# samyak0210/ViNet

Measured on AMD Instinct MI355X. Metric: clips/sec training (32x224x384 bf16), higher is better.
Workload: dtype bf16; 1 GPU; ViNet DHF1K training, 32x224x384 bf16, 192 clip(s)/GPU/step, kldiv + fused Adam, 1xMI355X; global_batch=192, local_batch=192, parallelism=dp1

## Files before the change

include/vinet_hip.h:

```cpp
#ifndef VINET_HIP_H
#define VINET_HIP_H

#include <stddef.h>
#include <stdint.h>

#ifdef __cplusplus
extern "C" {
#endif

#define VINET_ABI_VERSION 16

enum { VINET_F32 = 0, VINET_BF16 = 1,
       VINET_F32S = 2 };
enum { VINET_ACT_NONE = 0, VINET_ACT_RELU = 1, VINET_ACT_SIGMOID = 2 };
enum { VINET_CONV_GENERIC = 0, VINET_CONV_STEM = 1 };

typedef struct VinetTensor {
  void* ptr;
  int32_t B, T, H, W, C;
  int32_t ld;
  int64_t sB;
} VinetTensor;

typedef struct VinetAffine {
// ... 50 lines not shown
  VinetTensor x;
  VinetTensor dy;
  int32_t sT, sH, sW;
  int32_t ntaps;
  const int32_t* taps;
  float* dw;
  int32_t Kp;
  VinetAffine pre;
  int32_t tline;
  int32_t tpad;
  const void* bnb_z;
  int32_t bnb_ld;
  int64_t bnb_sB;
  VinetAffine bnb_fwd;
  const float* bnb_mean;
  const float* bnb_invstd;
  const float* bnb_c1;
  const float* bnb_c2;
  int32_t max_cus;
} VinetWgradDesc;

int vinet_conv3d_wgrad(const VinetWgradDesc* desc, void* stream);
int vinet_conv3d_wgrad_fuses_bn_bwd(const VinetWgradDesc* desc);
int vinet_conv3d_wgrad_kernel_name(const VinetWgradDesc* desc, char* buf, int32_t n);

int vinet_pack_weights(const float* w, int32_t N, int32_t Cin, int32_t ntaps, int32_t transpose, int32_t stem,
                       int32_t dtype, void* out, void* stream);

int vinet_pack_weights_multi(const int64_t* table, int32_t njobs, int64_t total, int32_t dtype, void* stream);
int vinet_unpack_wgrad(float* dw, int32_t N, int32_t Cin, int32_t ntaps, int32_t stem, int32_t flags,
                       float* grad, void* stream);
int vinet_unpack_wgrad_multi(const int64_t* table, int32_t njobs, int64_t total, int32_t flags, void* stream);

int vinet_import_ncdhw(const float* src, int64_t sb, int64_t sc, int64_t st, int64_t sh, int64_t sw, int32_t C,
                       const VinetTensor* dst, int32_t dst_dtype, void* stream);
int vinet_import_ncdhw_pad(const float* src, int64_t sb, int64_t sc, int64_t st, int64_t sh, int64_t sw, int32_t C,
                           int32_t Hs, int32_t Ws, int32_t pad_top, int32_t pad_left, const VinetTensor* dst,
                           int32_t dst_dtype, void* stream);
int vinet_export_ncdhw(const VinetTensor* src, int32_t src_dtype, VinetAffine pre, float* dst, int64_t sb, int64_t sc,
                       int64_t st, int64_t sh, int64_t sw, int32_t accumulate, void* stream);
int vinet_copy_affine(const VinetTensor* src, int32_t src_dtype, VinetAffine pre, const VinetTensor* dst,
                      int32_t dst_dtype, int32_t accumulate, void* stream);

int vinet_bn_finalize(const float* partials, int32_t rows, int32_t C, int32_t ld, double count, const float* gamma,
                      const float* beta, float eps, float momentum, float* running_mean, float* running_var,
                      float* mean, float* invstd, float* scale, float* shift, void* stream);
// ... 170 lines not shown
```

vinet_amd/_lib.py:

```python
import ctypes as C
import os

HERE = os.path.dirname(os.path.abspath(__file__))
LIB_PATH = os.environ.get("VINET_LIB") or os.path.join(HERE, "libvinet_hip.so")

F32, BF16 = 0, 1
F32S = 2
ACT_NONE, ACT_RELU, ACT_SIGMOID = 0, 1, 2
CONV_GENERIC, CONV_STEM = 0, 1
TK_MMA_F32, TK_MMA_BF16X3, TK_MMA_BF16 = 0, 1, 2
ABI_VERSION = 16


class CTensor(C.Structure):
    _fields_ = [("ptr", C.c_void_p), ("B", C.c_int32), ("T", C.c_int32), ("H", C.c_int32), ("W", C.c_int32),
                ("C", C.c_int32), ("ld", C.c_int32), ("sB", C.c_int64)]


class CAffine(C.Structure):
    _fields_ = [("scale", C.c_void_p), ("shift", C.c_void_p), ("relu", C.c_int32)]


class CConvDesc(C.Structure):
    _fields_ = [("dtype", C.c_int32), ("out_dtype", C.c_int32), ("mode", C.c_int32), ("x", CTensor), ("y", CTensor),
# ... 28 lines not shown
                ("L", C.c_int32), ("train", C.c_int32), ("p", C.c_float), ("eps", C.c_float), ("seed", C.c_uint64),
                ("step", C.c_void_p), ("pe", C.c_void_p), ("params", C.POINTER(C.c_void_p)), ("grads", C.POINTER(C.c_void_p)),
                ("ws", C.c_void_p), ("ws_bytes", C.c_int64), ("masks", C.c_void_p)]


class CTokenEncoderDesc(C.Structure):
    _fields_ = list(CTransformerDesc._fields_)


_vp, _i32, _i64, _f32, _f64 = C.c_void_p, C.c_int32, C.c_int64, C.c_float, C.c_double
_PT, _PC, _PW, _PP = C.POINTER(CTensor), C.POINTER(CConvDesc), C.POINTER(CWgradDesc), C.POINTER(CPoolDesc)
_PX = C.POINTER(CTransformerDesc)
_PK = C.POINTER(CTokenEncoderDesc)

SIGNATURES = {
    "vinet_conv3d": [_PC, _vp],
    "vinet_conv3d_tile_m": [_PC],
    "vinet_conv3d_stats_rows": [_PC],
    "vinet_conv3d_applies_pre_once": [_PC],
    "vinet_conv3d_splitk_bytes": [_PC],
    "vinet_conv3d_kernel_name": [_PC, C.c_char_p, _i32],
    "vinet_conv3d_wgrad": [_PW, _vp],
    "vinet_conv3d_wgrad_kernel_name": [_PW, C.c_char_p, _i32],
    "vinet_pack_weights": [_vp, _i32, _i32, _i32, _i32, _i32, _i32, _vp, _vp],
    "vinet_unpack_wgrad": [_vp, _i32, _i32, _i32, _i32, _i32, _vp, _vp],
    "vinet_import_ncdhw": [_vp, _i64, _i64, _i64, _i64, _i64, _i32, _PT, _i32, _vp],
    "vinet_import_ncdhw_pad": [_vp, _i64, _i64, _i64, _i64, _i64, _i32, _i32, _i32, _i32, _i32, _PT, _i32, _vp],
    "vinet_export_ncdhw": [_PT, _i32, CAffine, _vp, _i64, _i64, _i64, _i64, _i64, _i32, _vp],
    "vinet_copy_affine": [_PT, _i32, CAffine, _PT, _i32, _i32, _vp],
    "vinet_bn_finalize": [_vp, _i32, _i32, _i32, _f64, _vp, _vp, _f32, _f32, _vp, _vp, _vp, _vp, _vp, _vp, _vp],
    "vinet_bn_fold": [_vp, _vp, _vp, _vp, _vp, _f32, _i32, _vp, _vp, _vp, _vp],
    "vinet_channel_stats": [_PT, _i32, _vp, _vp],
    "vinet_stats_rows": [_PT],
    "vinet_bn_bwd_reduce": [_PT, _PT, _i32, CAffine, _vp, _vp, _vp, _vp],
    "vinet_conv3d_wgrad_fuses_bn_bwd": [_PW],
    "vinet_conv3d_fuses_dgrad_phases": [_PC],
    "vinet_conv3d_bn_bwd_stats_rows": [_PC],
    "vinet_bn_partials_fold": [_vp, _i32, _i32, _vp, _i32, _vp],
    "vinet_bn_bwd_finalize": [_vp, _i32, _i32, _i32, _f64, _vp, _i32, _vp, _vp, _vp, _vp, _vp, _vp],
    "vinet_bn_bwd_apply": [_PT, _PT, _i32, CAffine, _vp, _vp, _vp, _vp, _PT, _vp],
    "vinet_bn_bwd_apply_split": [_PT, _PT, CAffine, _vp, _vp, _vp, _vp, _PT, _PT, _PT, _vp],
    "vinet_bn_bwd_pool_ok": [_PP, _PT, _PT, _PT, _i32],
    "vinet_bn_bwd_reduce_pool": [_PP, _PT, _vp, _PT, _i32, _PT, _i32, CAffine, _vp, _vp, _vp, _vp],
    "vinet_bn_bwd_apply_pool": [_PP, _PT, _vp, _PT, _i32, _PT, _i32, CAffine, _vp, _vp, _vp, _vp, _PT, _vp],
    "vinet_act_bwd": [_PT, _i32, _PT, _i32, _i32, _PT, _i32, _vp],
    "vinet_channel_sum": [_PT, _i32, _vp, _i32, _vp, _i32, _vp],
# ... 133 lines not shown
```

vinet_amd/csrc/conv_wgrad.hip:

```cpp
#include "conv_host.h"

struct WgradArgs {
  const char* x;
  const char* dy;
  float* dw;
  const int4* taps;
  const float* in_scale;
  const float* in_shift;
  int in_relu;
  int Ti, Hi, Wi, Cin, ldx;
  long sBx;
  int To, Ho, Wo, N, ldy;
  long sBy;
  int sT, sH, sW;
  int ntaps, Kp, M;
  int tilesN, tilesC, splitK, chunks_per_split, nchunks;
  int use_tr;
  FastDiv dW, dH, dT;
};

VN_DEV void wg_split_pair(float x0, float x1, uint32_t& hi, uint32_t& lo) {
  hi = cvt_pk_bf16_f32(x0, x1);
  lo = cvt_pk_bf16_f32(x0 - __uint_as_float(hi << 16), x1 - __uint_as_float(hi & 0xffff0000u));
}
// ... 225 lines not shown
}

static bool wgrad_use_dma(const VinetWgradDesc* d) {
  const bool pre_ok = !d->pre.scale || (d->pre.relu && d->pre.shift);
  return g_vinet_opt_wgrad_dma && d->dtype == VINET_BF16 && d->mode == VINET_CONV_GENERIC && pre_ok &&
         !(d->pre.relu && !d->pre.scale);
}

WgradRoute vinet_wgrad_route(const VinetWgradDesc* d) {
  if (vinet_wgrad_use_skinny(d)) return {WGRAD_SKINNY};
  if (vinet_wgrad_use_rs(d)) return {WGRAD_RS};
  if (vinet_wgrad_use_hs(d)) return {WGRAD_HS};
  if (vinet_wgrad_use_ts(d)) return {WGRAD_TS};
  if (vinet_wgrad_use_tf(d)) return {WGRAD_TF};
  if (!wgrad_use_dma(d)) return {WGRAD_GENERIC};
  return {vinet_wgrad_use_pp(d) ? WGRAD_PP : WGRAD_DMA};
}

extern "C" int vinet_conv3d_wgrad_kernel_name(const VinetWgradDesc* d, char* buf, int32_t n) {
  if (!d || !buf || n <= 0) return -1;
  const char* pre = d->pre.scale ? "pre" : "plain";
  switch (vinet_wgrad_route(d).kind) {
    case WGRAD_SKINNY: snprintf(buf, n, "wgrad_skinny_kernel"); break;
    case WGRAD_RS: snprintf(buf, n, "conv_wgrad_rs_kernel<W%d,%s>", d->dy.W, vinet_wgrad_rs_four_wave(d) ? "4w" : "8w"); break;
    case WGRAD_HS: snprintf(buf, n, d->bnb_z ? "conv_wgrad_hs_kernel<bn_bwd>" : "conv_wgrad_hs_kernel"); break;
    case WGRAD_TS: snprintf(buf, n, "conv_wgrad_ts_kernel<%s>", pre); break;
    case WGRAD_TF: snprintf(buf, n, "conv_wgrad_tf_kernel<%s>", pre); break;
    case WGRAD_PP: snprintf(buf, n, "conv_wgrad_pp_kernel<%s,%d>", pre, vinet_wgrad_pp_rows(d->dy.C)); break;
    case WGRAD_DMA: return vinet_wgrad_dma_name(d, buf, n);
    case WGRAD_GENERIC: snprintf(buf, n, "conv_wgrad_kernel<%s,%d>", d->dtype == VINET_BF16 ? "bf16" : (d->dtype == VINET_F32S ? "float/split" : "float"), d->mode); break;
  }
  return 0;
}

extern "C" int vinet_conv3d_wgrad_fuses_bn_bwd(const VinetWgradDesc* d) {
  return d && d->bnb_z && vinet_wgrad_route(d).kind == WGRAD_HS ? 1 : 0;
}

static int vinet_launch_wgrad_generic(const VinetWgradDesc* d, hipStream_t s) {
  WgradArgs a;
  a.x = (const char*)d->x.ptr; a.dy = (const char*)d->dy.ptr; a.dw = d->dw; a.taps = (const int4*)d->taps;
  a.in_scale = d->pre.scale; a.in_shift = d->pre.shift; a.in_relu = d->pre.relu;
  a.Ti = d->x.T; a.Hi = d->x.H; a.Wi = d->x.W; a.Cin = d->x.C; a.ldx = d->x.ld; a.sBx = d->x.sB;
  a.To = d->dy.T; a.Ho = d->dy.H; a.Wo = d->dy.W; a.N = d->dy.C; a.ldy = d->dy.ld; a.sBy = d->dy.sB;
  a.sT = d->sT; a.sH = d->sH; a.sW = d->sW;
  a.ntaps = d->ntaps; a.Kp = d->Kp;
  const long M = (long)d->dy.B * d->dy.T * d->dy.H * d->dy.W;
  VN_CHECK_ARG(M < (1L << 31), "wgrad: M too large");
  a.M = (int)M;
  a.tilesN = vn_div_up(a.N, 64);
  a.tilesC = vn_div_up(d->mode == VINET_CONV_STEM ? 32 : a.Cin, 64);
  a.nchunks = vn_div_up(M, 32);
  const long base_blocks = (long)a.tilesN * a.tilesC * a.ntaps;
  long sk = (2048 + base_blocks - 1) / base_blocks;
  if (sk > a.nchunks / 4) sk = a.nchunks / 4;
  if (sk < 1) sk = 1;
  if (sk > 4096) sk = 4096;
  a.chunks_per_split = vn_div_up(a.nchunks, sk);
  a.splitK = vn_div_up(a.nchunks, a.chunks_per_split);
// ... 44 lines not shown
```

vinet_amd/csrc/options.h:

```cpp
#pragma once
#define VN_OPTIONS(VN_OPT) \
  VN_OPT(dma,          1, "LDS-DMA conv kernel (conv_dma) where legal; 0 = the register-staged kernel") \
  VN_OPT(dma3,         1, "LDS-DMA kernel for the split-bf16 form (conv_dma3); 0 = the register-staged kernel") \
  VN_OPT(pp,           1, "256x256x64 ping-pong conv kernel: 0 off, 1 heuristic, 2 force, 3 / 4 force the 256- / 192-wide shape") \
  VN_OPT(pp_pw_kt,     8, "ping-pong kernel on pointwise layers from this many K tiles of 64 (16 = as for every other layer)") \
  VN_OPT(pw,           1, "pointwise streaming kernel (conv_pw) for 1x1x1 convs and their data gradients: 0 off, 1 heuristic, 2 also on small grids (tests)") \
  VN_OPT(pw_maxtn,     4, "pointwise kernel: at most this many column tiles (each re-reads x)") \
  VN_OPT(ht,           1, "halo-tile conv kernels (conv_ht): 0 off, 1 heuristic, 2 every eligible conv (tests)") \
  VN_OPT(ht3,          1, "halo-tile kernels for the split-bf16 form; 0 = conv_dma3 everywhere") \
  VN_OPT(ht_minhw,     28 * 48, "halo tiles, spatial mode: smallest H x W the heuristic takes") \
  VN_OPT(ht_t,         1, "temporal mode of the halo-tile kernel for (3,1,1) / stride-1 convs; 0 off") \
  VN_OPT(ht_t_minhw,   14 * 24, "halo tiles, temporal mode: smallest H x W the heuristic takes") \
  VN_OPT(ht_pre,       0, "halo tiles, spatial mode, on inputs with a pending BatchNorm + ReLU: 1 on") \
  VN_OPT(conv_hs,      1, "strip-streaming kernel of the folded stem (conv_hs): 0 off, 1 heuristic, 2 every eligible shape (tests)") \
  VN_OPT(conv_hs_segs, 1, "conv_hs: row segments for launches on small grids; 0 = whole strips only") \
  VN_OPT(conv_ts,      1, "frame-streaming temporal 64 -> 64 kernels (conv_ts, conv_tsd): 0 off, 1 heuristic, 2 every eligible shape (tests)") \
  VN_OPT(conv_ts_segs, 1, "conv_ts: frame segments for launches on small grids; 0 = whole patches only") \
  VN_OPT(splitk,       1, "split-K on grids that cannot fill the chip: 0 off, 1 on, n >= 2 = minimum K chunks (of 32) per split") \
  VN_OPT(sk_tile,      7, "tiles of long-K small-grid convs whose caller lends split-K scratch: bit 0 128x192, bit 1 128x128, bit 2 / 3 128x64 / 256x64") \
  VN_OPT(n64_tile,     0, "tuning: 64-wide layers on 128x64 (1) or 64x64 (2) tiles instead of 256x64") \
  VN_OPT(n64_kmax,     64, "64-wide outputs: 128-row tiles up to this many K steps of 32 (0 = never)") \
  VN_OPT(n128_tile,    0, "tuning: 128-wide layers on 128x128 (1) or 64x128 (2) tiles instead of 256x128") \
  VN_OPT(n128_kmax,    64, "128-wide outputs: 128-row tiles up to this many K steps of 32 (0 = never)") \
  VN_OPT(n192_tile,    1, "128x192 tiles for N % 192 == 0 instead of 256x96: 0 off, 1 heuristic, 2 also on small grids (tests)") \
  VN_OPT(tperm,        0, "t-fastest M-tile order (L2 reuse across temporal taps): 1 on") \
  VN_OPT(bnb_epi,      1, "BatchNorm-backward partial sums out of the shared conv epilogue; 0 = only the fused temporal data gradient") \
  VN_OPT(wgrad_dma,    1, "LDS-DMA multi-tap weight-gradient kernel where legal; 0 = the register-staged kernel") \
  VN_OPT(wgrad_tg,     0, "tuning: taps per group in the LDS-DMA weight gradient (0 = heuristic)") \
  VN_OPT(wgrad_tr,     1, "hardware transpose reads in the register-staged weight gradient; 0 = scalar LDS reads") \
  VN_OPT(wgrad_pp,     1, "256x256x64 ping-pong weight gradient: 0 off, 1 heuristic, 2 force, 3 / 4 force the 256- / 192-row tile") \
  VN_OPT(wgrad_pp_cap, 1, "the ping-pong weight gradient honours VinetWgradDesc::max_cus; 0 = always the whole chip") \
  VN_OPT(wgrad_ts,     1, "frame-streaming weight gradient of temporal 64 -> 64 convs: 0 off, 1 heuristic, 2 every eligible shape (tests)") \
  VN_OPT(wgrad_ts_cap, 0, "the frame-streaming weight gradient honours VinetWgradDesc::max_cus: 1 on") \
  VN_OPT(wgrad_hs,     1, "strip-streaming weight gradient of the folded stem: 0 off, 1 heuristic, 2 every eligible shape (tests)") \
  VN_OPT(wgrad_rs,     1, "row-streaming weight gradient of 1x3x3 convs: 0 off, 1 heuristic, 2 every eligible shape (tests)") \
  VN_OPT(wgrad_rs4,    1, "row-streaming weight gradient: the four-wave form for W = 24, 48, 32, 64, 96; 0 = the eight-wave kernels") \
  VN_OPT(wgrad_tf,     1, "temporal-tap weight gradient (wgrad_tf): 0 off, 1 heuristic, 2 every eligible shape (tests)") \
  VN_OPT(wgrad_skinny, 1, "weight gradient of pointwise convs with 8 output channels: 0 off, 1 heuristic, 2 every eligible shape (tests)") \
  VN_OPT(bn_lean,      1, "register-lean bf16 BatchNorm-backward kernels: 0 = the generic 8-channel forms, 1 = register-lean") \
  VN_OPT(bn_rows,      1024, "cap on the workgroups (= partial rows) of a channel reduction (clamped to >= 1)") \
  VN_OPT(reduce_il,    1, "channel reductions: blocks interleave rounds over one window; 0 = one contiguous range per block") \
  VN_OPT(reduce_small, 1, "tensors of <= 64 voxels take channel_reduce_small_kernel; 0 off") \
  VN_OPT(pack_tiled,   1, "LDS-tiled multi-tensor pack / unpack; 0 = the element-wise kernels") \
  VN_OPT(pool_lds,     1, "LDS halo-tile 3x3x3/s1 max-pool forward (C % 64 == 0): 0 off, 1 large tensors, 2 always") \
  VN_OPT(pool_pk,      1, "bf16: packed 32-bit-key form of the LDS halo-tile pool; 0 = the fp32-compare kernel") \
  VN_OPT(pool_twalk,   1, "T-walking 3x3x3/s1 max-pool backward: 0 off, 1 large tensors, 2 always (any value above 3 too), 3 conditional-load form.  The forward's 8-channel T-walking kernel (kT 3, sT 1) reads it too: >= 2 forces it on small tensors, 0 does NOT switch it off") \
  VN_OPT(pool_blk,     1, "strided max-pool backward per 2x2 input block; 0 off") \
  VN_OPT(up_blk,       1, "8-channel upsample kernels (forward per 2x2 output block); 0 off") \
  VN_OPT(auc_ws,       0, "AUC-Judd sorts and counts in the caller's workspace whatever the number of fixations: 1 on (tests); 0 = in LDS up to 4096 fixations") \
  VN_OPT(sauc_ws,      0, "shuffled AUC reads the other-fixation list from the caller's workspace whatever its length: 1 on (tests); 0 = staged in LDS up to 8192 locations")

#define VN_OPT_DECLARE(name, dflt, text) extern int g_vinet_opt_##name;
VN_OPTIONS(VN_OPT_DECLARE)
```

vinet_amd/csrc/wgrad_rs.hip:

```cpp
#include "conv_host.h"

__device__ __attribute__((aligned(64))) uint4 g_vinet_zero_page_rs[4];

struct WgradRsArgs {
  const char* x;
  const char* dy;
  float* dw;
  long sBx, sBy;
  int Ti, To, H, W, ldx, ldy;
  int kT, cchunks, nchunks, Kp, N, Cin;
  int items, workers;
  FastDiv dTo;
  float* dbg;
};

#ifdef VINET_CONV_TIMING
static float* g_wrs_dbg = nullptr;
extern "C" void vinet_debug_wrs_ptr(float* p) { g_wrs_dbg = p; }
#endif
VN_DEV int wrs_swz(int r) { return (((r >> 1) & 1) | (((r >> 3) & 1) << 1)) << 1; }

template <int KS>
__global__ __launch_bounds__(512, 1) void conv_wgrad_rs_kernel(const WgradRsArgs a) {
  constexpr int W = KS * 32, RP = W + 2;
  constexpr int XROW = RP * 128, DROW = W * 128;
  constexpr int NPC = W * 8;
  constexpr int PPT = (NPC + 511) / 512;
  extern __shared__ __attribute__((aligned(16))) char smem[];
  char* ring = smem;
  char* dyb = smem + 3 * XROW;
  const int tid = threadIdx.x, lane = tid & 63, wave = __builtin_amdgcn_readfirstlane(tid >> 6);
  const int groups = a.kT * a.cchunks * a.nchunks;
  const int lid = xcd_remap((int)blockIdx.x, (int)gridDim.x);
  const int grp = lid % groups, worker = lid / groups;
  const int n0 = (grp % a.nchunks) * 64;
  const int gc = grp / a.nchunks;
// ... 344 lines not shown
    }
  }
#ifdef VINET_CONV_TIMING
  if (a.dbg && (tid & 63) == 0) {
    float* o = a.dbg + ((long)blockIdx.x * 8 + wave) * 8;
    o[0] = (float)(__builtin_amdgcn_s_memtime() - tm_start); o[1] = (float)tm_pro; o[2] = (float)tm_mma; o[3] = (float)tm_b1;
    o[4] = (float)tm_wr; o[5] = (float)tm_b2; o[6] = (float)tm_steps; o[7] = (float)tm_items;
  }
#endif
  mfma_drain();
#pragma unroll
  for (int t = 0; t < 9; ++t)
#pragma unroll
    for (int i = 0; i < 2; ++i)
#pragma unroll
      for (int r = 0; r < 4; ++r) {
        const int n = (nh * 2 + i) * 16 + (lane >> 4) * 4 + r, c = c0 + ct * 16 + (lane & 15);
        if (n0 + n < a.N && c < a.Cin) atomicAdd(a.dw + ((long)(kt * 9 + t) * a.N + n0 + n) * (long)a.Kp + c, acc[t][i][r]);
      }
}

constexpr int wrs_gcd(int a, int b) { return b == 0 ? a : wrs_gcd(b, a % b); }
template <int V> struct WrsIC { static constexpr int value = V; };

template <int KS, int WW>
__global__ __launch_bounds__(256, 1) void conv_wgrad_rs4_kernel(const WgradRsArgs a) {
  constexpr int P = KS * 32, R = P / WW, RING = 2 * R + 2, U = RING / wrs_gcd(R, RING);
  static_assert(R * WW == P && R >= 1 && WW % 8 == 0, "whole rows per step, 8-position DMA pieces inside one row");
  constexpr int XROW = (WW + 2) * 128, DROW = P * 128;
  constexpr int PPT = KS;
  extern __shared__ __attribute__((aligned(16))) char smem[];
  char* ring = smem;
  char* dyb = smem + RING * XROW;
  const int tid = threadIdx.x, lane = tid & 63, ct = __builtin_amdgcn_readfirstlane(tid >> 6);
  const int groups = a.kT * a.cchunks * a.nchunks;
  const int lid = xcd_remap((int)blockIdx.x, (int)gridDim.x);
  const int grp = lid % groups, worker = lid / groups;
  const int n0 = (grp % a.nchunks) * 64;
  const int gc = grp / a.nchunks;
  const int kt = gc / a.cchunks, c0 = (gc - kt * a.cchunks) * 64;
  const int l_chunk = tid & 7;
  const int H = a.H;
  const char* zero = (const char*)g_vinet_zero_page_rs;

  int xo[PPT], yo[PPT];
  int pr_[PPT], pw0_[PPT];
#pragma unroll
  for (int j = 0; j < PPT; ++j) {
    const int pos0 = j * 32 + ct * 8, pos = pos0 + (lane >> 3);
    const int pr = pos0 / WW, pw = pos - pr * WW;
    pr_[j] = pr; pw0_[j] = pos0 - pr * WW;
    const int xc = l_chunk ^ wrs_swz(pw + 1), dc = l_chunk ^ wrs_swz(pos);
    xo[j] = (pw * a.ldx + c0 + (c0 + xc * 8 < a.Cin ? xc * 8 : 0)) * 2;
    yo[j] = (pos * a.ldy + n0 + (n0 + dc * 8 < a.N ? dc * 8 : 0)) * 2;
  }
  auto dma = [&](const char* base, int off, char* dst) {
    __builtin_amdgcn_global_load_lds((const __attribute__((address_space(1))) void*)(base + (unsigned)off),
                                     (__attribute__((address_space(3))) void*)dst, 16, 0, 0);
  };
  for (int i = tid; i < RING * 2 * 8; i += 256) {
    const int row = i / 16, side = (i >> 3) & 1, ch = i & 7;
    *(uint4*)(ring + row * XROW + (side ? (WW + 1) * 128 : 0) + ch * 16) = make_uint4(0, 0, 0, 0);
  }
  const int p = lane & 15, q = lane >> 4;
  int xs[KS][2][3], xwrap[KS][2], da[KS][2], ds[KS][2];
  const int db = (p & 3) >> 1;
#pragma unroll
  for (int ks = 0; ks < KS; ++ks)
#pragma unroll
    for (int h = 0; h < 2; ++h) {
      const int pos = ks * 32 + q * 8 + h * 4 + (p >> 2);
      const int fr = pos / WW, fw = pos - fr * WW;
      const int frl = fr - (ks * 32) / WW;
      const int col = ct * 16 + (p & 3) * 4;
#pragma unroll
      for (int kw = 0; kw < 3; ++kw) xs[ks][h][kw] = frl * XROW + (fw + kw) * 128 + (((col >> 3) ^ wrs_swz(fw + kw)) * 16) + (col & 7) * 2;
      xwrap[ks][h] = frl * RING * XROW;
      da[ks][h] = pos * 128 + ((p & 3) & 1) * 8;
      ds[ks][h] = wrs_swz(pos);
    }

  f32x4_v acc[9][4];
#pragma unroll
  for (int t = 0; t < 9; ++t)
#pragma unroll
    for (int i = 0; i < 4; ++i) acc[t][i] = (f32x4_v){0.f, 0.f, 0.f, 0.f};

  auto keep = [](uint4 v, bool on) -> uint4 {
    const uint32_t m = on ? 0xffffffffu : 0u;
    return make_uint4(v.x & m, v.y & m, v.z & m, v.w & m);
  };
  const unsigned lds0 = (unsigned)(size_t)(__attribute__((address_space(3))) char*)smem;
  auto tr_read = [](unsigned addr, auto offc) -> s16x4_v {
    s16x4_v r;
#ifdef VINET_WRS_NO_LDS
    asm volatile("" : "=v"(r) : "v"(addr));
#else
    asm volatile("ds_read_b64_tr_b16 %0, %1 offset:%2" : "=v"(r) : "v"(addr), "n"(decltype(offc)::value));
#endif
    return r;
  };
#ifdef VINET_CONV_TIMING
  unsigned long long tm_pro = 0, tm_mma = 0, tm_b1 = 0, tm_wr = 0, tm_b2 = 0, tm_steps = 0, tm_items = 0;
  const unsigned long long tm_start = __builtin_amdgcn_s_memtime();
#endif
  const int nsteps = (H + R - 1) / R;
  const bool cx_ok = c0 + l_chunk * 8 < a.Cin, dn_ok = n0 + l_chunk * 8 < a.N;
  const int cx_off = cx_ok ? c0 + l_chunk * 8 : 0, dn_off = dn_ok ? n0 + l_chunk * 8 : 0;

  for (int item = worker; item < a.items; item += a.workers) {
    const int b = (int)fdiv((uint32_t)item, a.dTo);
    const int to = item - b * a.To;
    const int t = to * a.kT + kt;
    WRS_T(t_item0);
    const char* xi = a.x + ((long)b * a.sBx + (long)t * H * WW * a.ldx) * 2;
    const char* di = a.dy + ((long)b * a.sBy + (long)to * H * WW * a.ldy) * 2;
    const char* xb = xi + cx_off * 2;
    const char* db_ = di + dn_off * 2;
    const long xrowb = (long)WW * a.ldx * 2, drowb = (long)WW * a.ldy * 2;
    const char* xnext = xi + (long)(R + 1) * xrowb;
    const char* dnext = di + (long)R * drowb;
    long prx[PPT];
#pragma unroll
    for (int j = 0; j < PPT; ++j) prx[j] = (long)pr_[j] * xrowb;

    for (int e = tid; e < (R + 1) * WW * 8; e += 256) {
      const int pos = e >> 3, ch = e & 7;
      const int y = pos / WW, w = pos - y * WW;
      uint4 v = *(const uint4*)(xb + (long)(y < H ? pos : 0) * a.ldx * 2);
      v = keep(v, y < H && cx_ok);
      *(uint4*)(ring + (y + 1) * XROW + (w + 1) * 128 + ((ch ^ wrs_swz(w + 1)) * 16)) = v;
    }
    for (int e = tid; e < WW * 8; e += 256)
      *(uint4*)(ring + ((e >> 3) + 1) * 128 + (((e & 7) ^ wrs_swz((e >> 3) + 1)) * 16)) = make_uint4(0, 0, 0, 0);
    for (int e = tid; e < P * 8; e += 256) {
      const int pos = e >> 3, ch = e & 7;
      const bool in = pos / WW < H && dn_ok;
      const uint4 v = *(const uint4*)(db_ + (long)(in ? pos : 0) * a.ldy * 2);
      *(uint4*)(dyb + pos * 128 + ((ch ^ wrs_swz(pos)) * 16)) = keep(v, in);
    }
    __syncthreads();

#ifdef VINET_CONV_TIMING
    tm_pro += __builtin_amdgcn_s_memtime() - t_item0; ++tm_items;
#endif
    auto step = [&](auto uc, int st) {
      constexpr int SB = (decltype(uc)::value * R) % RING;
      WRS_T(t_s0);
      const int h0 = st * R;
      auto issue_dma = [&](int j) {
        char* dn = dyb + ((st + 1) & 1) * DROW;
        const bool xin = h0 + R + 1 + pr_[j] < H, din = h0 + R + pr_[j] < H;
        int sl = SB + R + 2 + pr_[j]; sl -= sl >= RING ? RING : 0;
        const char* xsrc = xnext + prx[j];
        xsrc = xin ? xsrc : zero;
        const char* dsrc = din ? dnext : zero;
        dma(xsrc, xo[j] & -(int)xin, ring + sl * XROW + (pw0_[j] + 1) * 128);
        dma(dsrc, yo[j] & -(int)din, dn + (j * 32 + ct * 8) * 128);
      };
      const unsigned dt = lds0 + RING * XROW + (st & 1) * DROW;
      union Frag { bf16x8_v v; s16x4_v h[2]; };
      Frag fa[4], fb[2][3];
      auto read_dy = [&](int ks) {
#pragma unroll
        for (int i = 0; i < 4; ++i)
#pragma unroll
          for (int h = 0; h < 2; ++h) fa[i].h[h] = tr_read(dt + da[ks][h] + (((2 * i + db) ^ ds[ks][h]) << 4), WrsIC<0>{});
      };
      auto read_x = [&](int buf, auto ksc, auto khc) {
        constexpr int ks = decltype(ksc)::value, kh = decltype(khc)::value;
        constexpr int f0 = (ks * 32) / WW;
        constexpr bool straddle = (ks * 32 + 31) / WW != f0;
        constexpr int slotA = (SB + f0 + kh) % RING;
        constexpr bool wraps = straddle && slotA + 1 == RING;
#pragma unroll
        for (int kw = 0; kw < 3; ++kw)
#pragma unroll
          for (int h = 0; h < 2; ++h)
            fb[buf][kw].h[h] = tr_read(lds0 + (wraps ? xs[ks][h][kw] - xwrap[ks][h] : xs[ks][h][kw]), WrsIC<slotA * XROW>{});
      };
      read_dy(0);
      read_x(0, WrsIC<0>{}, WrsIC<0>{});
      __builtin_amdgcn_sched_barrier(0);
      auto batch = [&](auto bc) {
        constexpr int b3 = decltype(bc)::value, ks = b3 / 3, kh = b3 % 3;
        if constexpr (b3 + 1 < KS * 3) {
          read_x((b3 + 1) & 1, WrsIC<(b3 + 1) / 3>{}, WrsIC<(b3 + 1) % 3>{});
          asm volatile("s_waitcnt lgkmcnt(6)" ::: "memory");
        } else {
          asm volatile("s_waitcnt lgkmcnt(0)" ::: "memory");
        }
        __builtin_amdgcn_sched_barrier(0);
#pragma unroll
        for (int kw = 0; kw < 3; ++kw)
#pragma unroll
          for (int i = 0; i < 4; ++i) {
#ifdef VINET_WRS_NO_MMA
            asm volatile("" :: "v"(fa[i].v), "v"(fb[b3 & 1][kw].v));
#else
            mfma_bf16_acc(acc[kh * 3 + kw][i], fa[i].v, fb[b3 & 1][kw].v);
#endif
          }
        __builtin_amdgcn_sched_barrier(0);
        if constexpr (b3 < PPT) {
          issue_dma(b3);
          __builtin_amdgcn_sched_barrier(0);
        }
        if constexpr (kh == 2 && ks + 1 < KS) {
          read_dy(ks + 1);
          __builtin_amdgcn_sched_barrier(0);
        }
      };
      batch(WrsIC<0>{}); batch(WrsIC<1>{}); batch(WrsIC<2>{});
      if constexpr (KS > 1) { batch(WrsIC<3>{}); batch(WrsIC<4>{}); batch(WrsIC<5>{}); }
      if constexpr (KS > 2) { batch(WrsIC<6>{}); batch(WrsIC<7>{}); batch(WrsIC<8>{}); }
      WRS_T(t_s1);
      xnext += (long)R * xrowb; dnext += (long)R * drowb;
      asm volatile("s_waitcnt vmcnt(0)" ::: "memory");
      __syncthreads();
      WRS_T(t_s2);
#ifdef VINET_CONV_TIMING
      tm_mma += t_s1 - t_s0; tm_b1 += t_s2 - t_s1; ++tm_steps;
#endif
    };
    for (int st = 0; st < nsteps; st += U) {
      step(WrsIC<0>{}, st);
      if constexpr (U > 1) { if (st + 1 < nsteps) step(WrsIC<1 % U>{}, st + 1); }
      if constexpr (U > 2) { if (st + 2 < nsteps) step(WrsIC<2 % U>{}, st + 2); }
      if constexpr (U > 3) { if (st + 3 < nsteps) step(WrsIC<3 % U>{}, st + 3); }
      if constexpr (U > 4) { if (st + 4 < nsteps) step(WrsIC<4 % U>{}, st + 4); }
      static_assert(U <= 5, "ring period");
    }
  }
#ifdef VINET_CONV_TIMING
  if (a.dbg && (tid & 63) == 0) {
    float* o = a.dbg + ((long)blockIdx.x * 4 + ct) * 8;
    o[0] = (float)(__builtin_amdgcn_s_memtime() - tm_start); o[1] = (float)tm_pro; o[2] = (float)tm_mma; o[3] = (float)tm_b1;
    o[4] = (float)tm_wr; o[5] = (float)tm_b2; o[6] = (float)tm_steps; o[7] = (float)tm_items;
  }
#endif
  mfma_drain();
#pragma unroll
  for (int t = 0; t < 9; ++t)
#pragma unroll
    for (int i = 0; i < 4; ++i)
#pragma unroll
      for (int r = 0; r < 4; ++r) {
        const int n = i * 16 + (lane >> 4) * 4 + r, c = c0 + ct * 16 + (lane & 15);
        if (n0 + n < a.N && c < a.Cin) atomicAdd(a.dw + ((long)(kt * 9 + t) * a.N + n0 + n) * (long)a.Kp + c, acc[t][i][r]);
      }
}

bool vinet_wgrad_use_rs(const VinetWgradDesc* d) {
  if (!g_vinet_opt_wgrad_rs || d->tline != 4 || d->dtype != VINET_BF16 || d->mode != VINET_CONV_GENERIC) return false;
  if (d->pre.scale || d->pre.relu || d->bnb_z) return false;
  const int kT = d->ntaps / 9;
  const bool shape = d->ntaps % 9 == 0 && kT >= 1 && d->sT == kT && d->sH == 1 && d->sW == 1 && d->dy.C % 8 == 0 && d->x.C % 8 == 0 && d->Kp >= d->x.C &&
                     kT * ((d->x.C + 63) / 64) * ((d->dy.C + 63) / 64) <= 256 &&
                     d->x.T == kT * d->dy.T && d->x.H == d->dy.H && d->x.W == d->dy.W && ((d->dy.W % 32 == 0 && d->dy.W <= 192) || d->dy.W == 48 || d->dy.W == 24) && d->dy.H >= 2 &&
                     d->x.ld % 8 == 0 && d->dy.ld % 8 == 0 && d->x.sB % 8 == 0 && d->dy.sB % 8 == 0 && ((uintptr_t)d->x.ptr % 16) == 0 &&
                     ((uintptr_t)d->dy.ptr % 16) == 0;
  if (!shape) return false;
  if (g_vinet_opt_wgrad_rs >= 2) return true;
  return (long)d->dy.B * d->dy.T >= 64 && d->dy.H >= 8;
}

bool vinet_wgrad_rs_four_wave(const VinetWgradDesc* d) {
  const int W = d->dy.W;
  return g_vinet_opt_wgrad_rs4 && (W == 24 || W == 48 || W == 32 || W == 64 || W == 96);
}

int vinet_launch_wgrad_rs(const VinetWgradDesc* d, hipStream_t s) {
  WgradRsArgs a;
  a.x = (const char*)d->x.ptr; a.dy = (const char*)d->dy.ptr; a.dw = d->dw;
  a.sBx = d->x.sB; a.sBy = d->dy.sB;
  a.Ti = d->x.T; a.To = d->dy.T; a.H = d->dy.H; a.W = d->dy.W; a.ldx = d->x.ld; a.ldy = d->dy.ld;
  a.kT = d->ntaps / 9; a.cchunks = (d->x.C + 63) / 64; a.nchunks = (d->dy.C + 63) / 64; a.Kp = d->Kp; a.N = d->dy.C; a.Cin = d->x.C;
  a.items = d->dy.B * a.To;
  a.dTo = make_fastdiv((uint32_t)a.To);
  a.dbg = nullptr;
#ifdef VINET_CONV_TIMING
  a.dbg = g_wrs_dbg;
#endif
  const int groups = a.kT * a.cchunks * a.nchunks;
  int workers = vn_wgrad_cus(d) / groups;
  if (workers < 1) workers = 1;
  if (workers > a.items) workers = a.items;
  a.workers = workers;
  if (vinet_wgrad_rs_four_wave(d)) {
    const int ks4 = (a.W == 24 || a.W == 48) ? 3 : a.W / 32;
    const int rows = ks4 * 32 / a.W;
    const int smem4 = (2 * rows + 2) * (a.W + 2) * 128 + 2 * ks4 * 32 * 128;
    int w4 = 2 * vn_wgrad_cus(d) / groups;
    if (w4 < 1) w4 = 1;
    if (w4 > a.items) w4 = a.items;
    a.workers = w4;
    auto launch4 = [&](auto kern) -> int {
      static bool attr_done[64] = {false};
      int dev = 0;
      (void)hipGetDevice(&dev);
      if (!attr_done[dev & 63]) {
        hipError_t e = hipFuncSetAttribute((const void*)kern, hipFuncAttributeMaxDynamicSharedMemorySize, 96 * 1024);
        if (e != hipSuccess) { vinet_set_error("hipFuncSetAttribute(wgrad_rs4): %s", hipGetErrorString(e)); return (int)e; }
        attr_done[dev & 63] = true;
      }
      hipLaunchKernelGGL(kern, dim3(groups * w4), dim3(256), smem4, s, a);
      return vn_launch_status("conv_wgrad_rs4");
    };
    if (a.W == 48) return launch4(conv_wgrad_rs4_kernel<3, 48>);
    if (a.W == 24) return launch4(conv_wgrad_rs4_kernel<3, 24>);
    if (a.W == 32) return launch4(conv_wgrad_rs4_kernel<1, 32>);
    if (a.W == 64) return launch4(conv_wgrad_rs4_kernel<2, 64>);
    return launch4(conv_wgrad_rs4_kernel<3, 96>);
  }
  const bool multi = a.W == 48 || a.W == 24;
  const int ks = multi ? 3 : a.W / 32;
  const int ringrows = multi ? 96 / a.W + 2 : 3;
  const int smem = ringrows * (a.W + 2) * 128 + 2 * ks * 32 * 128;
  auto launch = [&](auto kern) -> int {
    if (smem > 64 * 1024) {
      static bool attr_done[64] = {false};
      int dev = 0;
      (void)hipGetDevice(&dev);
      if (!attr_done[dev & 63]) {
        hipError_t e = hipFuncSetAttribute((const void*)kern, hipFuncAttributeMaxDynamicSharedMemorySize, smem);
        if (e != hipSuccess) { vinet_set_error("hipFuncSetAttribute(wgrad_rs): %s", hipGetErrorString(e)); return (int)e; }
        attr_done[dev & 63] = true;
      }
    }
    hipLaunchKernelGGL(kern, dim3(groups * workers), dim3(512), smem, s, a);
    return vn_launch_status("conv_wgrad_rs");
// ... 11 lines not shown
```

vinet_amd/engine.py:

```python
import collections
import ctypes as C
import itertools
import math
import os
import weakref

import torch

from . import _lib as L

F32, BF16 = L.F32, L.BF16
F32S = L.F32S
TORCH_DT = {F32: torch.float32, BF16: torch.bfloat16}
ESIZE = {F32: 4, BF16: 2}
EG = {F32: 4, BF16: 8}

_DEFAULT_DTYPE = BF16
_WEIGHTS_EPOCH = 0
_UNPACK_TABLES = {}
_SIDE_STREAMS = {}

_CONFIG = dict(
    WGRAD_SIDE_STREAM=True,
    WGRAD_CUS=208,
# ... 1039 lines not shown

def conv_forward(ctx, plan, x, bn=None, act=L.ACT_NONE, dst=None, out_dt=None, n_pad=None):
    note_reader(ctx, x)
    want_plain = (MATERIALIZE_NT and x.scale is not None and ctx.dt != L.F32 and x.fold is None and not plan.stem and
                  plan.N * plan.ntaps >= MATERIALIZE_NT and x.v.dt == ctx.dt)
    xv = x.v
    folded = plan.stem and x.fold is not None
    if folded:
        odims = xv.T, (x.fold[0] - 1) // 2 + 1, (x.fold[1] - 1) // 2 + 1
    else:
        odims = plan.out_dims(xv.T, xv.H, xv.W)
    Ny = plan.N if n_pad is None else n_pad
    if dst is None:
        dst = Act(View.alloc(xv.B, odims[0], odims[1], odims[2], Ny, ctx.dt if out_dt is None else out_dt, xv.device))
    out = dst.v
    given = (dst.scale, dst.shift, dst.mean, dst.invstd)
    dst.mean = dst.invstd = None
    assert (out.B, out.T, out.H, out.W, out.C) == (xv.B,) + tuple(odims) + (Ny,), "conv output view mismatch"
    taps, ntaps = plan.folded_taps(ctx.device) if folded else plan.fwd_taps(ctx.device)
    w = plan.packed(ctx, False)
    d = _conv_desc(ctx, L.CONV_STEM if (plan.stem and not folded) else L.CONV_GENERIC, xv, out, odims,
                   (1, 2, 1) if folded else plan.s, (1, 1, 1), (0, 0, 0), ntaps, taps, w, plan.kp(False), x.affine(),
                   plan.N if Ny != plan.N else 0, plan.promise("fwd", folded), 0)
    if want_plain and not ctx.lib.vinet_conv3d_applies_pre_once(C.byref(d)):
        x = materialize(ctx, x)
        xv = x.v
        d.x, d.pre = xv.ct(), x.affine()
    M = xv.B * odims[0] * odims[1] * odims[2]
    es = ESIZE[ctx.dt]
    tag, work = _conv_prof(ctx, d, "fwd", plan, xv, M, es, ESIZE[out.dt], es)

    train_bn = bn is not None and ctx.training
    keep = {}
    res = dst
    res.needs_grad = True
    if bn is None:
        _run_conv(ctx, d, None, _ptr(plan.bias), act, None, tag, work, splitk=True)
        res.scale = res.shift = None
        res.relu = False
        res.act_out = act
    elif train_bn:
        rows = ctx.lib.vinet_conv3d_stats_rows(C.byref(d))
        stats = ctx.f32(rows * 2 * plan.N)
        _run_conv(ctx, d, None, _ptr(plan.bias), L.ACT_NONE, stats.data_ptr(), tag, work)
        scale, shift, mean, invstd = (ctx.f32(plan.N) if g is None else g for g in given)
        if rows >= 1024:
            per = (rows + 255) // 256
# ... 90 lines not shown
        hi = View.alloc(v.B, v.T, v.H, v.W, v.C, BF16, v.device)
        lo = View.alloc(v.B, v.T, v.H, v.W, v.C, BF16, v.device)
        ctx.call("vinet_split_bf16", C.byref(v.ct()), aff, C.byref(hi.ct()), C.byref(lo.ct()), ctx.stream)
        out.append((hi, lo))
    if dy_planes is not None:
        out.append(dy_planes)
    return out


def _wgrad_desc(ctx, plan, x, dy, dw=None):
    folded = plan.stem and x.fold is not None
    taps, ntaps = plan.folded_taps(ctx.device) if folded else plan.fwd_taps(ctx.device)
    wd = L.CWgradDesc()
    wd.dtype, wd.mode = ctx.cdt, (L.CONV_STEM if (plan.stem and not folded) else L.CONV_GENERIC)
    wd.x, wd.dy = x.v.ct(), dy.ct()
    wd.sT, wd.sH, wd.sW = (1, 2, 1) if folded else plan.s
    wd.ntaps, wd.taps, wd.dw, wd.Kp = ntaps, taps.data_ptr(), (dw.data_ptr() if dw is not None else None), plan.kp(False)
    wd.pre = x.affine()
    wd.tline, wd.tpad = plan.promise("wgrad", folded)
    wd._keep = taps
    return wd


def _conv_backward(ctx, plan, x, res, bn, act, train_bn, keep, M):
    pool = _take_pool_rec(res, bn, train_bn, x)
    dz = res.grad_view()
    assert res.is_grad_ready(), "conv backward reached before any consumer produced a gradient"
    fused_bnb = dy_planes = None
    if bn is not None:
        sums = _bn_backward_sums(ctx, res, bn, train_bn, keep, M, dz, pool)
        dy, fused_bnb, dy_planes = _bn_backward_apply(ctx, plan, x, res, keep, dz, pool, *sums)
    else:
        dy = _act_backward(ctx, res, act, dz)
    if plan.bias is not None and plan.bias.requires_grad:
        _bias_grad(ctx, plan, dy)
    if plan.wants_wgrad():
        for w_ in plan.grad_targets():
            _param_grad(w_)
        _schedule_wgrad(ctx, _WgradJob(ctx, plan, x, dy, M, bn is None, fused_bnb, dy_planes))
    if x.needs_grad:
        _data_grad(ctx, plan, x, res.v, dy, M)


def _bn_backward_sums(ctx, res, bn, train_bn, keep, M, dz, pool):
    out, Ny = res.v, res.v.C
    mean, invstd = keep["mean"], keep["invstd"]
# ... 395 lines not shown
```

Baseline: 720.5 clips/s.

## Fuse pending BatchNorm+ReLU into the four-wave row-streaming weight-gradient kernel

```diff
diff --git a/include/vinet_hip.h b/include/vinet_hip.h
--- a/include/vinet_hip.h
+++ b/include/vinet_hip.h
@@ -96,6 +96,7 @@
 
 int vinet_conv3d_wgrad(const VinetWgradDesc* desc, void* stream);
 int vinet_conv3d_wgrad_fuses_bn_bwd(const VinetWgradDesc* desc);
+int vinet_conv3d_wgrad_applies_pre_once(const VinetWgradDesc* desc);
 int vinet_conv3d_wgrad_kernel_name(const VinetWgradDesc* desc, char* buf, int32_t n);
 
 int vinet_pack_weights(const float* w, int32_t N, int32_t Cin, int32_t ntaps, int32_t transpose, int32_t stem,
diff --git a/vinet_amd/_lib.py b/vinet_amd/_lib.py
--- a/vinet_amd/_lib.py
+++ b/vinet_amd/_lib.py
@@ -74,6 +74,7 @@
     "vinet_conv3d_kernel_name": [_PC, C.c_char_p, _i32],
     "vinet_conv3d_wgrad": [_PW, _vp],
     "vinet_conv3d_wgrad_kernel_name": [_PW, C.c_char_p, _i32],
+    "vinet_conv3d_wgrad_applies_pre_once": [_PW],
     "vinet_pack_weights": [_vp, _i32, _i32, _i32, _i32, _i32, _i32, _vp, _vp],
     "vinet_unpack_wgrad": [_vp, _i32, _i32, _i32, _i32, _i32, _vp, _vp],
     "vinet_import_ncdhw": [_vp, _i64, _i64, _i64, _i64, _i64, _i32, _PT, _i32, _vp],
diff --git a/vinet_amd/csrc/conv_wgrad.hip b/vinet_amd/csrc/conv_wgrad.hip
--- a/vinet_amd/csrc/conv_wgrad.hip
+++ b/vinet_amd/csrc/conv_wgrad.hip
@@ -271,7 +271,7 @@
   const char* pre = d->pre.scale ? "pre" : "plain";
   switch (vinet_wgrad_route(d).kind) {
     case WGRAD_SKINNY: snprintf(buf, n, "wgrad_skinny_kernel"); break;
-    case WGRAD_RS: snprintf(buf, n, "conv_wgrad_rs_kernel<W%d,%s>", d->dy.W, vinet_wgrad_rs_four_wave(d) ? "4w" : "8w"); break;
+    case WGRAD_RS: snprintf(buf, n, "conv_wgrad_rs_kernel<W%d,%s%s>", d->dy.W, vinet_wgrad_rs_four_wave(d) ? "4w" : "8w", d->pre.scale ? ",pre" : ""); break;
     case WGRAD_HS: snprintf(buf, n, d->bnb_z ? "conv_wgrad_hs_kernel<bn_bwd>" : "conv_wgrad_hs_kernel"); break;
     case WGRAD_TS: snprintf(buf, n, "conv_wgrad_ts_kernel<%s>", pre); break;
     case WGRAD_TF: snprintf(buf, n, "conv_wgrad_tf_kernel<%s>", pre); break;
@@ -284,6 +284,10 @@
 
 extern "C" int vinet_conv3d_wgrad_fuses_bn_bwd(const VinetWgradDesc* d) {
   return d && d->bnb_z && vinet_wgrad_route(d).kind == WGRAD_HS ? 1 : 0;
+}
+
+extern "C" int vinet_conv3d_wgrad_applies_pre_once(const VinetWgradDesc* d) {
+  return d && d->pre.scale && vinet_wgrad_route(d).kind == WGRAD_RS ? 1 : 0;
 }
 
 static int vinet_launch_wgrad_generic(const VinetWgradDesc* d, hipStream_t s) {
diff --git a/vinet_amd/csrc/options.h b/vinet_amd/csrc/options.h
--- a/vinet_amd/csrc/options.h
+++ b/vinet_amd/csrc/options.h
@@ -34,7 +34,7 @@
   VN_OPT(wgrad_ts_cap, 0, "the frame-streaming weight gradient honours VinetWgradDesc::max_cus: 1 on") \
   VN_OPT(wgrad_hs,     1, "strip-streaming weight gradient of the folded stem: 0 off, 1 heuristic, 2 every eligible shape (tests)") \
   VN_OPT(wgrad_rs,     1, "row-streaming weight gradient of 1x3x3 convs: 0 off, 1 heuristic, 2 every eligible shape (tests)") \
-  VN_OPT(wgrad_rs4,    1, "row-streaming weight gradient: the four-wave form for W = 24, 48, 32, 64, 96; 0 = the eight-wave kernels") \
+  VN_OPT(wgrad_rs4,    1, "row-streaming weight gradient: the four-wave form for W = 24, 48, 32, 64, 96, also on inputs with a pending BatchNorm + ReLU (applied once per staged element, in the ring); 2 = the four-wave form on plain inputs only (pending inputs fall to the LDS-DMA multi-tap kernel); 0 = the eight-wave kernels") \
   VN_OPT(wgrad_tf,     1, "temporal-tap weight gradient (wgrad_tf): 0 off, 1 heuristic, 2 every eligible shape (tests)") \
   VN_OPT(wgrad_skinny, 1, "weight gradient of pointwise convs with 8 output channels: 0 off, 1 heuristic, 2 every eligible shape (tests)") \
   VN_OPT(bn_lean,      1, "register-lean bf16 BatchNorm-backward kernels: 0 = the generic 8-channel forms, 1 = register-lean") \
diff --git a/vinet_amd/csrc/wgrad_rs.hip b/vinet_amd/csrc/wgrad_rs.hip
--- a/vinet_amd/csrc/wgrad_rs.hip
+++ b/vinet_amd/csrc/wgrad_rs.hip
@@ -12,6 +12,8 @@
   int items, workers;
   FastDiv dTo;
   float* dbg;
+  const float* pre_scale;
+  const float* pre_shift;
 };
 
 #ifdef VINET_CONV_TIMING
@@ -402,9 +404,10 @@
 
 constexpr int wrs_gcd(int a, int b) { return b == 0 ? a : wrs_gcd(b, a % b); }
 template <int V> struct WrsIC { static constexpr int value = V; };
-
-template <int KS, int WW>
-__global__ __launch_bounds__(256, 1) void conv_wgrad_rs4_kernel(const WgradRsArgs a) {
+typedef __attribute__((ext_vector_type(4))) uint32_t wrs_u32x4;
+
+template <int KS, int WW, bool PRE>
+__device__ __forceinline__ void wgrad_rs4_body(const WgradRsArgs a) {
   constexpr int P = KS * 32, R = P / WW, RING = 2 * R + 2, U = RING / wrs_gcd(R, RING);
   static_assert(R * WW == P && R >= 1 && WW % 8 == 0, "whole rows per step, 8-position DMA pieces inside one row");
   constexpr int XROW = (WW + 2) * 128, DROW = P * 128;
@@ -425,6 +428,9 @@
 
   int xo[PPT], yo[PPT];
   int pr_[PPT], pw0_[PPT];
+  constexpr int NV = WW == 24 ? PPT : 1;
+  int xch[PPT];
+  unsigned xlive[PPT];
 #pragma unroll
   for (int j = 0; j < PPT; ++j) {
     const int pos0 = j * 32 + ct * 8, pos = pos0 + (lane >> 3);
@@ -433,14 +439,34 @@
     const int xc = l_chunk ^ wrs_swz(pw + 1), dc = l_chunk ^ wrs_swz(pos);
     xo[j] = (pw * a.ldx + c0 + (c0 + xc * 8 < a.Cin ? xc * 8 : 0)) * 2;
     yo[j] = (pos * a.ldy + n0 + (n0 + dc * 8 < a.N ? dc * 8 : 0)) * 2;
+    xch[j] = xc; xlive[j] = c0 + xc * 8 < a.Cin ? 0xffffffffu : 0u;
   }
   auto dma = [&](const char* base, int off, char* dst) {
-    __builtin_amdgcn_global_load_lds((const __attribute__((address_space(1))) void*)(base + (unsigned)off),
-                                     (__attribute__((address_space(3))) void*)dst, 16, 0, 0);
+    if constexpr (PRE) lds_dma16_asm(base + (unsigned)off, dst);
+    else __builtin_amdgcn_global_load_lds((const __attribute__((address_space(1))) void*)(base + (unsigned)off),
+                                          (__attribute__((address_space(3))) void*)dst, 16, 0, 0);
   };
   for (int i = tid; i < RING * 2 * 8; i += 256) {
     const int row = i / 16, side = (i >> 3) & 1, ch = i & 7;
     *(uint4*)(ring + row * XROW + (side ? (WW + 1) * 128 : 0) + ch * 16) = make_uint4(0, 0, 0, 0);
+  }
+  float* const aff = (float*)(smem + RING * XROW + 2 * DROW);
+  f32x2_v sc2[NV][4], sh2[NV][4];
+  if constexpr (PRE) {
+    if (tid < 64) {
+      const bool in = c0 + tid < a.Cin;
+      aff[tid] = in ? a.pre_scale[c0 + tid] : 0.f;
+      aff[64 + tid] = in ? a.pre_shift[c0 + tid] : 0.f;
+    }
+    __syncthreads();
+#pragma unroll
+    for (int v = 0; v < NV; ++v)
+#pragma unroll
+      for (int e = 0; e < 4; ++e) {
+        const float* sp = aff + xch[v] * 8 + e * 2;
+        sc2[v][e] = (f32x2_v){sp[0], sp[1]};
+        sh2[v][e] = (f32x2_v){sp[64], sp[65]};
+      }
   }
   const int p = lane & 15, q = lane >> 4;
   int xs[KS][2][3], xwrap[KS][2], da[KS][2], ds[KS][2];
@@ -476,7 +502,7 @@
 #ifdef VINET_WRS_NO_LDS
     asm volatile("" : "=v"(r) : "v"(addr));
 #else
-    asm volatile("ds_read_b64_tr_b16 %0, %1 offset:%2" : "=v"(r) : "v"(addr), "n"(decltype(offc)::value));
+    asm volatile("ds_read_b64_tr_b16 %0, %1 offset:%2" : "=v"(r) : "v"(addr), "n"(decltype(offc)::value) : "memory");
 #endif
     return r;
   };
@@ -504,10 +530,22 @@
 #pragma unroll
     for (int j = 0; j < PPT; ++j) prx[j] = (long)pr_[j] * xrowb;
 
+    f32x2_v ps2[4], ph2[4];
+    if constexpr (PRE) {
+#pragma unroll
+      for (int e = 0; e < 4; ++e) {
+        const float* sp = aff + l_chunk * 8 + e * 2;
+        ps2[e] = (f32x2_v){sp[0], sp[1]};
+        ph2[e] = (f32x2_v){sp[64], sp[65]};
+      }
+    }
     for (int e = tid; e < (R + 1) * WW * 8; e += 256) {
       const int pos = e >> 3, ch = e & 7;
       const int y = pos / WW, w = pos - y * WW;
       uint4 v = *(const uint4*)(xb + (long)(y < H ? pos : 0) * a.ldx * 2);
+      if constexpr (PRE)
+        v = make_uint4(pre_relu_pair(v.x, ps2[0], ph2[0]), pre_relu_pair(v.y, ps2[1], ph2[1]), pre_relu_pair(v.z, ps2[2], ph2[2]),
+                       pre_relu_pair(v.w, ps2[3], ph2[3]));
       v = keep(v, y < H && cx_ok);
       *(uint4*)(ring + (y + 1) * XROW + (w + 1) * 128 + ((ch ^ wrs_swz(w + 1)) * 16)) = v;
     }
@@ -528,6 +566,8 @@
       constexpr int SB = (decltype(uc)::value * R) % RING;
       WRS_T(t_s0);
       const int h0 = st * R;
+      unsigned pdst[PPT], pmask[PPT];
+      wrs_u32x4 pv[PPT];
       auto issue_dma = [&](int j) {
         char* dn = dyb + ((st + 1) & 1) * DROW;
         const bool xin = h0 + R + 1 + pr_[j] < H, din = h0 + R + pr_[j] < H;
@@ -537,6 +577,10 @@
         const char* dsrc = din ? dnext : zero;
         dma(xsrc, xo[j] & -(int)xin, ring + sl * XROW + (pw0_[j] + 1) * 128);
         dma(dsrc, yo[j] & -(int)din, dn + (j * 32 + ct * 8) * 128);
+        if constexpr (PRE) {
+          pdst[j] = lds0 + sl * XROW + (pw0_[j] + 1) * 128 + lane * 16;
+          pmask[j] = xlive[j] & -(unsigned)xin;
+        }
       };
       const unsigned dt = lds0 + RING * XROW + (st & 1) * DROW;
       union Frag { bf16x8_v v; s16x4_v h[2]; };
@@ -569,6 +613,10 @@
           asm volatile("s_waitcnt lgkmcnt(6)" ::: "memory");
         } else {
           asm volatile("s_waitcnt lgkmcnt(0)" ::: "memory");
+          if constexpr (PRE) {
+#pragma unroll
+            for (int j = 0; j < PPT; ++j) asm volatile("" : "+v"(pv[j]));
+          }
         }
         __builtin_amdgcn_sched_barrier(0);
 #pragma unroll
@@ -580,8 +628,27 @@
 #else
             mfma_bf16_acc(acc[kh * 3 + kw][i], fa[i].v, fb[b3 & 1][kw].v);
 #endif
+            if constexpr (PRE && b3 + 1 == KS * 3) {
+              const int n = kw * 4 + i;
+              if (n < 4 * PPT) {
+                const int j = n >> 2, e = n & 3;
+                pv[j][e] = pre_relu_pair(pv[j][e], sc2[NV == 1 ? 0 : j][e], sh2[NV == 1 ? 0 : j][e]) & pmask[j];
+                __builtin_amdgcn_sched_barrier(0);
+              }
+            }
           }
         __builtin_amdgcn_sched_barrier(0);
+        if constexpr (PRE && b3 + 1 == KS * 3) {
+#pragma unroll
+          for (int j = 0; j < PPT; ++j) asm volatile("ds_write_b128 %0, %1" ::"v"(pdst[j]), "v"(pv[j]) : "memory");
+          __builtin_amdgcn_sched_barrier(0);
+        }
+        if constexpr (PRE && b3 + 2 == KS * 3) {
+          asm volatile("s_waitcnt vmcnt(0)" ::: "memory");
+#pragma unroll
+          for (int j = 0; j < PPT; ++j) asm volatile("ds_read_b128 %0, %1" : "=&v"(pv[j]) : "v"(pdst[j]) : "memory");
+          __builtin_amdgcn_sched_barrier(0);
+        }
         if constexpr (b3 < PPT) {
           issue_dma(b3);
           __builtin_amdgcn_sched_barrier(0);
@@ -596,7 +663,8 @@
       if constexpr (KS > 2) { batch(WrsIC<6>{}); batch(WrsIC<7>{}); batch(WrsIC<8>{}); }
       WRS_T(t_s1);
       xnext += (long)R * xrowb; dnext += (long)R * drowb;
-      asm volatile("s_waitcnt vmcnt(0)" ::: "memory");
+      if constexpr (PRE) asm volatile("s_waitcnt vmcnt(0) lgkmcnt(0)" ::: "memory");
+      else asm volatile("s_waitcnt vmcnt(0)" ::: "memory");
       __syncthreads();
       WRS_T(t_s2);
 #ifdef VINET_CONV_TIMING
@@ -631,9 +699,16 @@
       }
 }
 
+template <int KS, int WW>
+__global__ __launch_bounds__(256, 1) void conv_wgrad_rs4_kernel(const WgradRsArgs a) { wgrad_rs4_body<KS, WW, false>(a); }
+template <int KS, int WW>
+__global__ __launch_bounds__(256, 1) void conv_wgrad_rs4_pre_kernel(const WgradRsArgs a) { wgrad_rs4_body<KS, WW, true>(a); }
+
 bool vinet_wgrad_use_rs(const VinetWgradDesc* d) {
   if (!g_vinet_opt_wgrad_rs || d->tline != 4 || d->dtype != VINET_BF16 || d->mode != VINET_CONV_GENERIC) return false;
-  if (d->pre.scale || d->pre.relu || d->bnb_z) return false;
+  if (d->bnb_z) return false;
+  if ((d->pre.scale || d->pre.relu) &&
+      !(g_vinet_opt_wgrad_rs4 != 2 && d->pre.scale && d->pre.shift && d->pre.relu && vinet_wgrad_rs_four_wave(d))) return false;
   const int kT = d->ntaps / 9;
   const bool shape = d->ntaps % 9 == 0 && kT >= 1 && d->sT == kT && d->sH == 1 && d->sW == 1 && d->dy.C % 8 == 0 && d->x.C % 8 == 0 && d->Kp >= d->x.C &&
                      kT * ((d->x.C + 63) / 64) * ((d->dy.C + 63) / 64) <= 256 &&
@@ -659,6 +734,7 @@
   a.items = d->dy.B * a.To;
   a.dTo = make_fastdiv((uint32_t)a.To);
   a.dbg = nullptr;
+  a.pre_scale = d->pre.scale; a.pre_shift = d->pre.shift;
 #ifdef VINET_CONV_TIMING
   a.dbg = g_wrs_dbg;
 #endif
@@ -670,7 +746,8 @@
   if (vinet_wgrad_rs_four_wave(d)) {
     const int ks4 = (a.W == 24 || a.W == 48) ? 3 : a.W / 32;
     const int rows = ks4 * 32 / a.W;
-    const int smem4 = (2 * rows + 2) * (a.W + 2) * 128 + 2 * ks4 * 32 * 128;
+    const bool pre = d->pre.scale != nullptr;
+    const int smem4 = (2 * rows + 2) * (a.W + 2) * 128 + 2 * ks4 * 32 * 128 + (pre ? 512 : 0);
     int w4 = 2 * vn_wgrad_cus(d) / groups;
     if (w4 < 1) w4 = 1;
     if (w4 > a.items) w4 = a.items;
@@ -687,6 +764,13 @@
       hipLaunchKernelGGL(kern, dim3(groups * w4), dim3(256), smem4, s, a);
       return vn_launch_status("conv_wgrad_rs4");
     };
+    if (pre) {
+      if (a.W == 48) return launch4(conv_wgrad_rs4_pre_kernel<3, 48>);
+      if (a.W == 24) return launch4(conv_wgrad_rs4_pre_kernel<3, 24>);
+      if (a.W == 32) return launch4(conv_wgrad_rs4_pre_kernel<1, 32>);
+      if (a.W == 64) return launch4(conv_wgrad_rs4_pre_kernel<2, 64>);
+      return launch4(conv_wgrad_rs4_pre_kernel<3, 96>);
+    }
     if (a.W == 48) return launch4(conv_wgrad_rs4_kernel<3, 48>);
     if (a.W == 24) return launch4(conv_wgrad_rs4_kernel<3, 24>);
     if (a.W == 32) return launch4(conv_wgrad_rs4_kernel<1, 32>);
diff --git a/vinet_amd/engine.py b/vinet_amd/engine.py
--- a/vinet_amd/engine.py
+++ b/vinet_amd/engine.py
@@ -1085,7 +1085,7 @@
     d = _conv_desc(ctx, L.CONV_STEM if (plan.stem and not folded) else L.CONV_GENERIC, xv, out, odims,
                    (1, 2, 1) if folded else plan.s, (1, 1, 1), (0, 0, 0), ntaps, taps, w, plan.kp(False), x.affine(),
                    plan.N if Ny != plan.N else 0, plan.promise("fwd", folded), 0)
-    if want_plain and not ctx.lib.vinet_conv3d_applies_pre_once(C.byref(d)):
+    if want_plain and not (ctx.lib.vinet_conv3d_applies_pre_once(C.byref(d)) and _wgrad_keeps_pre_once(ctx, plan, x, out)):
         x = materialize(ctx, x)
         xv = x.v
         d.x, d.pre = xv.ct(), x.affine()
@@ -1222,6 +1222,11 @@
     return wd
 
 
+def _wgrad_keeps_pre_once(ctx, plan, x, out):
+    wd = _wgrad_desc(ctx, plan, x, out)
+    return wd.tline != 4 or bool(ctx.lib.vinet_conv3d_wgrad_applies_pre_once(C.byref(wd)))
+
+
 def _conv_backward(ctx, plan, x, res, bn, act, train_bn, keep, M):
     pool = _take_pool_rec(res, bn, train_bn, x)
     dz = res.grad_view()
```

Result: no change. 719.9 clips/s (-0.1%).
